# nicoRomeroCuruchet/DynamicProgramming

Hardware: AMD Instinct MI355X
Metric: state-action Bellman backups/sec (higher is better)
Workload: dtype f32; 1 GPU; double_pendulum_swingup 4D grid bins=80/dim (40960000 states) x 11 actions, gamma=0.999; step = 10 eval sweeps + 1 improve sweep = 860160000 backups; terminal states are counted in `value` (0 of 40960000: value_nonterminal leaves them out); states=40960000, nonterminal_states=40960000, actions=11, parallelism=state-range shards x1

## Files before the change

### dynamicprogramming_amd/_native.py

```python
from __future__ import annotations

import ctypes
import enum
import os
from pathlib import Path

import numpy as np

_PKG = Path(__file__).resolve().parent
LIB_PATH = _PKG / "libpi_mi355.so"
KERNEL_CACHE = Path(os.environ.get("PI_MI355_KERNEL_CACHE", str(_PKG / "_kcache")))

_f32p = ctypes.POINTER(ctypes.c_float)
_i32p = ctypes.POINTER(ctypes.c_int32)
_vp = ctypes.c_void_p

SIGNATURES = {
    "pi_abi_version": (ctypes.c_int, []),
    "pi_last_error": (ctypes.c_char_p, []),
    "pi_create": (_vp, [ctypes.c_int, ctypes.c_int, _i32p, _f32p, _f32p,
                        ctypes.POINTER(_f32p), _f32p, ctypes.c_int]),
    "pi_destroy": (None, [_vp]),
    "pi_compile": (ctypes.c_int, [_vp, ctypes.c_char_p, ctypes.c_char_p, ctypes.c_char_p,
                                  ctypes.c_size_t]),
# ... 63 lines not shown
ABI_VERSION = 12
_lib = None
_load_error: Exception | None = None


class Info(enum.IntEnum):
    N_STATES = 0
    N_ACTIONS = 1
    DIMS = 2
    EVAL_CPW = 3
    EVAL_VGPRS = 4
    IMPROVE_VGPRS = 5
    COMPUTE_UNITS = 6
    CACHE_HIT = 7
    IMPROVE_CPW = 8
    CACHED_GRAPHS = 9
    GRAPHS_ENABLED = 10
    EVAL_BLOCK = 11
    IMPROVE_BLOCK = 12
    RESIDENT_STATES_PER_THREAD = 13
    RESIDENT_ENABLED = 14
    DEBUG_CHECKS = 15
    LIVE_STATES = 16
    EVAL_LIST_ENTRIES = 17
    MEMORY_ORDER = 18
    FLOW_WORKGROUPS = 19
    RECIPROCAL_DIV = 20
    XCD_ENABLED = 30
    XCD_EVALUATIONS = 31
    XCD_FALLBACKS = 32
    WHOLE_RUNS = 33
    WHOLE_RUN_AVAILABLE = 34
    STRIP_STATES = 35


class Option(enum.IntEnum):
    EVAL_CPW = 0
    IMPROVE_CPW = 1
    GRAPHS = 2
    RESIDENT = 3
    MEMORY_ORDER = 4
    BUILD_PUSH = 5
    KEEP_LIVE_LIST = 6
    STRIP_STATES = 7
    XCD_RUN_FAILED = 8


class XcdFailure(enum.IntEnum):
    COUNT = 1
    SWITCH_OFF = 2


class CommInfo(enum.IntEnum):
    RANK = 0
    WORLD = 1
    TRANSPORT = 2
    PLAN = 3
    REACH_UNITS = 4
    ROW_EXACT = 5
    FUSED = 6
    PAIR_EXACT = 7
    FUSED_VALUES = 8
    FIRST_ENTRIES = 9
    INTERIOR_ENTRIES = 10


class Transport(enum.IntEnum):
    RCCL = 1
    IN_PROCESS = 2
    P2P = 3


class Plan(enum.IntEnum):
    NONE = 0
    ALLGATHER = 1
    HALO = 2


# ... 417 lines not shown
```

### dynamicprogramming_amd/csrc/pi_api.cpp

```cpp

#include "pi_internal.h"

#include <algorithm>
#include <cstdlib>

namespace pi {

static thread_local std::string g_error;

int fail(const std::string& msg) {
    g_error = msg;
    return 1;
}
const std::string& last_error() { return g_error; }

int env_int(const char* name, int dflt, int lo, int hi) {
    if (const char* e = std::getenv(name)) {
        const int v = std::atoi(e);
        if (v >= lo && v <= hi) return v;
    }
    return dflt;
}

void resolve_strip(pi_handle* h) {
    if (h->strip_mode >= 0) { h->strip_states = h->strip_mode; return; }
    h->strip_states = 0;
    if (h->D == 6 && h->n_states >= (int64_t(1) << 24)) {
        const int64_t sub = h->n_states / ((int64_t)h->shape[0] * h->shape[1]);
        h->strip_states = sub * std::max<int64_t>(1, ((int64_t(1) << 21) + sub / 2) / sub);
    }
}

void drop_graphs(pi_handle* h) {
    for (auto& g : h->graphs)
        if (g.exec) (void)hipGraphExecDestroy(g.exec);
    h->graphs.clear();
}

unsigned launch_blocks(int block, int64_t count, int cpw) {
    const int64_t chunks = (count + block - 1) / block;
    const int64_t groups = (chunks + cpw - 1) / cpw;
    const int64_t span = (groups + kXcds - 1) / kXcds;
    return (unsigned)std::max<int64_t>(span * kXcds, kXcds);
}

Grid2 plan_launch(const pi_handle* h, int block, int64_t first, int64_t count, int64_t total, int cpw, Sched* sc) {
    sc->cpw = cpw;
    sc->period = sc->phase = 0u;
    const int64_t group = (int64_t)block * cpw;
    const int64_t groups = ((count + block - 1) / block + cpw - 1) / cpw;
    if (h->strip_states > 0 && total > 0) {
        const double units = (double)h->strip_states * ((double)total / (double)h->n_states);
        const int64_t T = (int64_t)(units / (double)group + 0.5);
        if (T >= 16 && T < (int64_t(1) << 24) && groups > T) {
            const int64_t seg = (T + kXcds - 1) / kXcds;
            const int64_t phase = (first / group) % T;
            const int64_t periods = (groups + phase + T - 1) / T;
            if (periods <= 65535 && periods * T < (int64_t(1) << 31)) {
                sc->period = (unsigned)T;
                sc->phase = (unsigned)phase;
                return Grid2{(unsigned)(seg * kXcds), (unsigned)periods};
            }
        }
    }
    return Grid2{launch_blocks(block, count, cpw), 1u};
}

}

using namespace pi;

namespace {

unsigned int* delta_slots(pi_handle* h) { return h->d_slots; }
unsigned int* changed_slots(pi_handle* h) { return h->d_slots + kSlots; }

int zero_outputs(float* d_delta, uint32_t* d_changed, hipStream_t st) {
    if (d_delta) PI_HIP(hipMemsetAsync(d_delta, 0, sizeof(float), st));
    if (d_changed) PI_HIP(hipMemsetAsync(d_changed, 0, sizeof(uint32_t), st));
    return 0;
}

void free_device_state(pi_handle* h) {
    drop_graphs(h);
    if (h->module) (void)hipModuleUnload(h->module);
    if (h->module_push) (void)hipModuleUnload(h->module_push);
    for (void* p : {(void*)h->d_tab, (void*)h->d_slots, (void*)h->d_live, (void*)h->d_eval_list, (void*)h->d_eval_cursor,
                    h->d_flow, h->d_xcd})
        if (p) (void)hipFree(p);
}

int allocate_device_state(pi_handle* h) {
    h->num_cu = 256;
    if (h->device < 0) return 0;
    pi::DeviceGuard guard(h->device);
    hipDeviceProp_t prop;
    hipError_t e = hipGetDeviceProperties(&prop, h->device);
    if (e == hipSuccess && std::string(prop.gcnArchName).rfind(pi::kArch, 0) != 0)
        return fail(std::string("pi_create: device is ") + prop.gcnArchName + ", this library is built for gfx950 only");
    if (e == hipSuccess) e = hipMalloc((void**)&h->d_tab, h->tab.size() * sizeof(float));
    if (e == hipSuccess) e = hipMemcpy(h->d_tab, h->tab.data(), h->tab.size() * sizeof(float), hipMemcpyHostToDevice);
    if (e == hipSuccess) e = hipMalloc((void**)&h->d_slots, 2 * kSlots * sizeof(unsigned int));
    if (e == hipSuccess) e = hipMemset(h->d_slots, 0, 2 * kSlots * sizeof(unsigned int));
    if (e != hipSuccess) {
        free_device_state(h);
        return fail(std::string("pi_create: ") + hipGetErrorString(e));
    }
    h->num_cu = prop.multiProcessorCount;
    return 0;
}

void choose_dispatch(pi_handle* h) {
    const int D = h->D;
    const int64_t n = h->n_states;
    const bool big = D <= 4 && n >= (int64_t(1) << 24);
    auto block_knob = [](const char* name, int dflt) {
        const int v = env_int(name, dflt, 256, 1024);
        return (v % 64 == 0) ? v : dflt;
    };
    h->block_eval = block_knob("PI_MI355_EVAL_BLOCK", big ? 1024 : 256);
    h->block_improve = block_knob("PI_MI355_IMPROVE_BLOCK", big ? 512 : 256);
// ... 11 lines not shown
    h->resident_block = D == 2 ? 1024 : 512;
    h->resident_k = (n <= resident_max && env_int("PI_MI355_RESIDENT", 1, 0, 1))
                        ? (int)((n + h->resident_block - 1) / h->resident_block) : 0;
    const bool one_launch = env_int("PI_MI355_RESIDENT", 1, 0, 1) != 0 && env_int("PI_MI355_FLOW", 1, 0, 1) != 0;
    const bool xcd_wanted = one_launch && D == 2 && n <= (int64_t)env_int("PI_MI355_XCD_MAX", 1 << 16, 1 << 12, 1 << 17) && env_int("PI_MI355_XCD", 1, 0, 1) != 0;
    const int64_t flow_min = xcd_wanted ? std::min<int64_t>(resident_max, env_int("PI_MI355_XCD_MIN", 4096, 1024, 12288)) : resident_max;
    const int64_t flow_max = D <= 4 ? (int64_t(1) << 17) : 0;
    h->flow = one_launch && n > flow_min && n <= flow_max;
    h->xcd = h->flow && xcd_wanted;
    h->xcd_ring = env_int("PI_MI355_XCD_RING", 64, 4, 1024);
    h->xcd_states = (int)(((n + 31) / 32 + 31) / 32 * 32);
}

int build_eval_graph(pi_handle* h, float* Va, float* Vb, const int32_t* policy, const uint8_t* term,
                     int64_t s_begin, int64_t s_end, float gamma, int n_sweeps, float* d_delta,
                     hipGraphExec_t* out) {
    hipGraph_t graph;
    PI_HIP(hipGraphCreate(&graph, 0));
    hipGraphNode_t prev = nullptr;
    int rc = 0;
    for (int i = 0; i < n_sweeps && !rc; ++i)
        rc = pi::launch_eval(h, (i & 1) ? Vb : Va, (i & 1) ? Va : Vb, policy, term, s_begin, s_end, gamma,
                             i == n_sweeps - 1 && d_delta, pi::LaunchTo(graph, &prev), i >= 1);
    if (!rc) rc = pi::finalize(h, d_delta, nullptr, pi::LaunchTo(graph, &prev));
    if (!rc && hipGraphInstantiate(out, graph, nullptr, nullptr, 0) != hipSuccess) rc = 1;
    (void)hipGraphDestroy(graph);
    if (rc) {
        (void)hipGetLastError();
        return fail("could not build the evaluation-sweep graph");
    }
    return 0;
}

}

int pi::check_ready(const pi_handle* h) {
    if (!h) return fail("null handle");
    if (h->device < 0) return fail("host-only handle (device = -1) cannot launch kernels");
    if (!h->module) return fail("pi_compile has not been called on this handle");
    return 0;
}

int pi::check_range(const pi_handle* h, int64_t s_begin, int64_t s_end) {
    if (s_begin < 0 || s_end < s_begin || s_end > h->n_states)
        return fail("state range [" + std::to_string(s_begin) + ", " + std::to_string(s_end) +
                    ") outside [0, " + std::to_string(h->n_states) + ")");
    return 0;
}

int pi::finalize(pi_handle* h, float* d_delta, uint32_t* d_changed, LaunchTo to) {
    if (!d_delta && !d_changed) return 0;
    PI_HIP(launch(h->f_finalize, {1, 1}, 64, to, d_delta ? delta_slots(h) : (unsigned int*)nullptr, d_delta,
                  d_changed ? changed_slots(h) : (unsigned int*)nullptr, d_changed));
    return 0;
}

int pi::launch_eval(pi_handle* h, const float* V, float* Vnew, const int32_t* policy, const uint8_t* term,
                int64_t s_begin, int64_t s_end, float gamma, bool want_delta, LaunchTo to, bool keep_terminals) {
    if (s_end == s_begin) return 0;
    Sched sc;
    const Grid2 blocks = plan_launch(h, h->block_eval, s_begin, s_end - s_begin, h->n_states, h->cpw_eval, &sc);
    PI_HIP(launch(h->f_eval, blocks, h->block_eval, to, V, Vnew, policy, term, (const float*)h->d_tab, (long long)s_begin,
                  (long long)s_end, gamma, want_delta ? delta_slots(h) : (unsigned int*)nullptr, sc, keep_terminals ? 1 : 0));
    return 0;
}

// ... 70 lines not shown
    if (!h) return;
    if (h->device >= 0) {
        pi::DeviceGuard guard(h->device);
        pi::release_comm(h);
        free_device_state(h);
    }
    delete h;
}

int pi_eval_sweep(pi_handle* h, const float* V, float* Vnew, const int32_t* policy,
                  const uint8_t* term, int64_t s_begin, int64_t s_end, float gamma,
                  float* d_delta, void* stream) {
    if (check_ready(h) || check_range(h, s_begin, s_end)) return 1;
    if (!V || !Vnew || !policy) return fail("null device pointer");
    if (V == Vnew) return fail("V and Vnew must be different buffers (Jacobi sweep)");
    pi::DeviceGuard guard(h->device);
    hipStream_t st = (hipStream_t)stream;
    if (s_end == s_begin) return zero_outputs(d_delta, nullptr, st);
    if (pi::launch_eval(h, V, Vnew, policy, term, s_begin, s_end, gamma, d_delta != nullptr, st)) return 1;
    return pi::finalize(h, d_delta, nullptr, st);
}

int pi_eval_sweeps(pi_handle* h, float* Va, float* Vb, const int32_t* policy,
                   const uint8_t* term, int64_t s_begin, int64_t s_end, float gamma,
                   int n_sweeps, float* d_delta, void* stream) {
    if (check_ready(h) || check_range(h, s_begin, s_end)) return 1;
    if (n_sweeps < 0) return fail("n_sweeps < 0");
    if (!Va || !Vb || !policy) return fail("null device pointer");
    if (Va == Vb) return fail("Va and Vb must be different buffers (Jacobi sweep)");
    if (n_sweeps == 0) return 0;
    pi::DeviceGuard guard(h->device);
    hipStream_t st = (hipStream_t)stream;
    if (s_end == s_begin) return zero_outputs(d_delta, nullptr, st);
    if (h->f_resident && h->use_resident && n_sweeps >= 2 && s_begin == 0 && s_end == h->n_states) {
        PI_HIP(launch(h->f_resident, {1, 1}, h->resident_block, st, Va, Vb, policy, term, (const float*)h->d_tab, gamma, n_sweeps,
                      d_delta,  0.0,  1,  (int*)nullptr,  (float*)nullptr));
        return 0;
    }
    if (h->use_graphs && n_sweeps >= 4 && s_end - s_begin <= (int64_t(1) << 20)) {
        pi::GraphEntry* hit = nullptr;
        for (auto& g : h->graphs)
            if (g.Va == Va && g.Vb == Vb && g.policy == policy && g.term == term &&
                g.d_delta == d_delta && g.s_begin == s_begin && g.s_end == s_end &&
                g.gamma == gamma && g.n_sweeps == n_sweeps)
                hit = &g;
        if (!hit) {
            hipGraphExec_t exec = nullptr;
            if (build_eval_graph(h, Va, Vb, policy, term, s_begin, s_end, gamma, n_sweeps, d_delta, &exec)) {
                h->use_graphs = false;
            } else {
                if (h->graphs.size() >= 16) {
                    auto lru = std::min_element(h->graphs.begin(), h->graphs.end(),
                                                [](const GraphEntry& a, const GraphEntry& b) { return a.stamp < b.stamp; });
                    (void)hipGraphExecDestroy(lru->exec);
                    h->graphs.erase(lru);
                }
                h->graphs.push_back({Va, Vb, policy, term, d_delta, s_begin, s_end, gamma, n_sweeps, exec, 0});
                hit = &h->graphs.back();
            }
        }
        if (hit) {
            hit->stamp = ++h->graph_clock;
            PI_HIP(hipGraphLaunch(hit->exec, st));
            return 0;
        }
    }
// ... 113 lines not shown
            if (v != 0) return fail("memory order: too many digits");
            std::vector<int32_t> shape(h->D);
            std::vector<float> lo(h->D), span(h->D), rcp(h->D), tab(h->tab.begin(), h->tab.begin() + h->n_actions);
            std::vector<int> fastdiv(h->D);
            std::vector<size_t> off(h->D);
            size_t at = (size_t)h->n_actions;
            for (int d = 0; d < h->D; ++d) { off[d] = at; at += (size_t)h->shape[d]; }
            for (int k = 0; k < h->D; ++k) {
                const int d = perm[k];
                shape[k] = h->shape[d]; lo[k] = h->lo[d]; span[k] = h->span[d]; rcp[k] = h->rcp[d]; fastdiv[k] = h->fastdiv[d];
                tab.insert(tab.end(), h->tab.begin() + off[d], h->tab.begin() + off[d] + h->shape[d]);
                h->mem_of_user[d] = k;
            }
            h->user_of_mem = perm;
            h->shape = shape; h->lo = lo; h->span = span; h->rcp = rcp; h->fastdiv = fastdiv; h->tab = tab;
            if (h->device >= 0) {
                pi::DeviceGuard guard(h->device);
                PI_HIP(hipMemcpy(h->d_tab, h->tab.data(), h->tab.size() * sizeof(float), hipMemcpyHostToDevice));
            }
            return 0;
        }
        case PI_OPTION_BUILD_PUSH:
            if (value == 0) return 0;
            return pi::ensure_push_module(h);
        case PI_OPTION_KEEP_LIVE_LIST:
            h->live_force = value != 0;
            return 0;
        case PI_OPTION_STRIP_STATES:
            if (value < -1 || value > h->n_states) return fail("strip period must be -1 (auto), 0 (off) or a number of states <= n");
            h->strip_mode = value;
            resolve_strip(h);
            drop_graphs(h);
            return 0;
        case PI_OPTION_XCD_RUN_FAILED:
            if (value != PI_XCD_FAILURE_COUNT && value != PI_XCD_FAILURE_SWITCH_OFF)
                return fail("option 8 takes 1 (count a failed whole run) or 2 (and switch the XCD-local kernel off)");
            if (++h->xcd_failed >= 2 || value == PI_XCD_FAILURE_SWITCH_OFF) h->xcd_off = true;
            return 0;
        default:
            return fail("unknown option");
    }
}

int pi_debug_report(pi_handle* h, uint32_t* out4) {
    if (pi::check_ready(h)) return 1;
    if (!out4) return fail("null argument");
    if (!h->debug_bounds) return fail("this handle's kernels were built without the checks: set PI_MI355_DEBUG=1 before pi_create");
    pi::DeviceGuard guard(h->device);
    hipDeviceptr_t words = nullptr;
    size_t bytes = 0;
    PI_HIP(hipModuleGetGlobal(&words, &bytes, h->module, "pi_debug_words"));
    if (bytes != 4 * sizeof(uint32_t)) return fail("pi_debug_words has an unexpected size");
    PI_HIP(hipDeviceSynchronize());
    PI_HIP(hipMemcpy(out4, words, bytes, hipMemcpyDeviceToHost));
    PI_HIP(hipMemset(words, 0, bytes));
    return 0;
}

int64_t pi_info(pi_handle* h, int what) {
    if (!h) return -1;
    switch (what) {
        case PI_INFO_N_STATES: return h->n_states;
        case PI_INFO_N_ACTIONS: return h->n_actions;
        case PI_INFO_DIMS: return h->D;
        case PI_INFO_EVAL_CPW: return h->cpw_eval;
        case PI_INFO_EVAL_VGPRS: return h->vgpr_eval;
        case PI_INFO_IMPROVE_VGPRS: return h->vgpr_improve;
        case PI_INFO_COMPUTE_UNITS: return h->num_cu;
        case PI_INFO_CACHE_HIT: return h->cache_hit ? 1 : 0;
        case PI_INFO_IMPROVE_CPW: return h->cpw_improve;
        case PI_INFO_CACHED_GRAPHS: return (int64_t)h->graphs.size();
        case PI_INFO_GRAPHS_ENABLED: return h->use_graphs ? 1 : 0;
        case PI_INFO_EVAL_BLOCK: return h->block_eval;
        case PI_INFO_IMPROVE_BLOCK: return h->block_improve;
        case PI_INFO_RESIDENT_STATES_PER_THREAD: return h->resident_k;
        case PI_INFO_RESIDENT_ENABLED: return h->use_resident ? 1 : 0;
        case PI_INFO_DEBUG_CHECKS: return h->debug_bounds ? 1 : 0;
        case PI_INFO_LIVE_STATES: return h->live_count;
        case PI_INFO_EVAL_LIST_ENTRIES: return h->eval_count < 0 ? 0 : h->eval_count;
        case PI_INFO_MEMORY_ORDER: {
            int64_t code = 0;
            for (int k = h->D - 1; k >= 0; --k) code = (code << 3) | h->user_of_mem[k];
            return code;
        }
        case PI_INFO_FLOW_WORKGROUPS:
            return h->f_flow ? (h->n_states + h->flow_block - 1) / h->flow_block : (h->flow && h->device < 0 ? 1 : 0);
        case PI_INFO_XCD_ENABLED: return h->f_xcd && !h->xcd_off ? 1 : 0;
        case PI_INFO_XCD_EVALUATIONS: return h->xcd_used;
        case PI_INFO_XCD_FALLBACKS: return h->xcd_failed;
        case PI_INFO_WHOLE_RUNS: return h->whole_runs;
        case PI_INFO_WHOLE_RUN_AVAILABLE: return (h->f_run_resident && h->use_resident) || (h->f_xcd && !h->xcd_off) ? 1 : 0;
        case PI_INFO_STRIP_STATES: return h->strip_states;
        default:
            if (what >= PI_INFO_RECIPROCAL_DIV && what < PI_INFO_RECIPROCAL_DIV + h->D)
                return h->fastdiv[what - PI_INFO_RECIPROCAL_DIV];
            return -1;
    }
}

}
```

### dynamicprogramming_amd/csrc/pi_compile.cpp

```cpp

#include "pi_internal.h"

#include <hip/hiprtc.h>

#include <cmath>
#include <cstdio>
#include <cstdlib>
#include <algorithm>
#include <cstring>
#include <fstream>
#include <map>
#include <mutex>
#include <sstream>
#include <sys/stat.h>
#include <unistd.h>

#ifndef PI_CSRC_DIR
#error "build with -DPI_CSRC_DIR=\"...\" and -DPI_INCLUDE_DIR=\"...\""
#endif
asm(".section .rodata\n"
    ".global pi_embedded_kernels\n"
    "pi_embedded_kernels:\n"
    ".incbin \"" PI_CSRC_DIR "/pi_sweep_kernels.hip\"\n"
    ".byte 0\n"
    ".global pi_embedded_onelaunch\n"
    "pi_embedded_onelaunch:\n"
    ".incbin \"" PI_CSRC_DIR "/pi_onelaunch_kernels.hip\"\n"
    ".byte 0\n"
    ".global pi_embedded_math\n"
    "pi_embedded_math:\n"
    ".incbin \"" PI_INCLUDE_DIR "/pi_math.h\"\n"
    ".byte 0\n"
    ".global pi_embedded_push\n"
    "pi_embedded_push:\n"
    ".incbin \"" PI_CSRC_DIR "/pi_push_kernels.hip\"\n"
    ".byte 0\n"
    ".text\n");

using pi::env_int;
using pi::fail;
using pi::kXcds;

namespace {

const char* const kCompileFlags[] = {"--offload-arch=gfx950", "-O3", "-ffp-contract=off",
                                     "-std=c++17"};

uint64_t fnv1a(const std::string& s, uint64_t h) {
    for (unsigned char c : s) {
        h ^= c;
        h *= 1099511628211ull;
    }
    return h;
}

float bits_to_float(uint32_t u) {
    float f;
    std::memcpy(&f, &u, 4);
    return f;
}
// ... 50 lines not shown
std::string build_source(const pi_handle* h, const char* dynamics_src) {
    std::ostringstream o;
    auto dec = [](int x) { return std::to_string(x); };
    auto list = [](const auto& v, auto fmt) { return pi::brace_list(v.data(), v.size(), fmt); };
    o << "// generated by libpi_mi355 for " << pi::kArch << "\n";
    o << "#define PI_BLOCK_EVAL " << h->block_eval << "\n";
    o << "#define PI_BLOCK_IMPROVE " << h->block_improve << "\n";
    o << "#define PI_RESIDENT_K " << h->resident_k << "\n";
    o << "#define PI_RESIDENT_BLOCK " << h->resident_block << "\n";
    if (h->flow) o << "#define PI_FLOW 1\n#define PI_FLOW_BLOCK " << h->flow_block << "\n";
    if (h->xcd) o << "#define PI_XCD 1\n#define PI_XCD_S " << h->xcd_states << "\n#define PI_XCD_RING " << h->xcd_ring
                  << "\n#define PI_XCD_HOST_CTL_WORDS " << pi::kXcdCtlWords << "\n";
    if (h->xcd && std::getenv("PI_MI355_XCD_FIRST_SLEEP")) o << "#define PI_XCD_FIRST_SLEEP " << env_int("PI_MI355_XCD_FIRST_SLEEP", 8, 0, 127) << "\n";
    if (h->xcd && std::getenv("PI_MI355_XCD_TIMING")) o << "#define PI_XCD_TIMING 1\n";
    if (h->debug_bounds) o << "#define PI_DEBUG_BOUNDS 1\n";
    o << "#define PI_D " << h->D << "\n";
    o << "#define PI_NA " << h->n_actions << "\n";
    o << "#define PI_GRID_INIT " << list(h->shape, dec) << "\n";
    o << "#define PI_LO_INIT " << list(h->lo, pi::hex_float) << "\n";
    o << "#define PI_SPAN_INIT " << list(h->span, pi::hex_float) << "\n";
    o << "#define PI_RCP_INIT " << list(h->rcp, pi::hex_float) << "\n";
    o << "#define PI_FASTDIV_INIT " << list(h->fastdiv, dec) << "\n";
    o << "#define PI_MEM_OF_INIT " << list(h->mem_of_user, dec) << "\n";
    o << pi_embedded_math << "\n";
    o << "#define sinf pi_sinf\n#define cosf pi_cosf\n#define fmodf pi_fmodf\n";
    o << "// ---- env plugin (user string) ----\n";
    o << dynamics_src << "\n";
    o << "// ---- sweep kernels ----\n";
    o << pi_embedded_kernels << "\n";
    if (h->resident_k > 0 || h->flow || h->xcd) {
        o << "// ---- one-launch kernels ----\n";
        o << pi_embedded_onelaunch << "\n";
    }
    return o.str();
}

int load_module(pi_handle* h, const std::vector<char>& image) {
    if (h->device < 0) return 0;
    pi::DeviceGuard guard(h->device);
    pi::drop_graphs(h);
    if (h->module) {
        PI_HIP(hipModuleUnload(h->module));
        h->module = nullptr;
    }
    if (h->module_push) {
        PI_HIP(hipModuleUnload(h->module_push));
        h->module_push = nullptr;
        h->f_eval_push = nullptr;
        h->f_reach_pairs = nullptr;
    }
    PI_HIP(hipModuleLoadData(&h->module, image.data()));
    PI_HIP(hipModuleGetFunction(&h->f_eval, h->module, "pi_eval_sweep_kernel"));
    PI_HIP(hipModuleGetFunction(&h->f_eval_live, h->module, "pi_eval_live_kernel"));
    PI_HIP(hipModuleGetFunction(&h->f_policy_list, h->module, "pi_policy_list_kernel"));
    PI_HIP(hipModuleGetFunction(&h->f_scan_slots, h->module, "pi_scan_slots_kernel"));
    PI_HIP(hipModuleGetFunction(&h->f_mask_list, h->module, "pi_mask_list_kernel"));
    PI_HIP(hipModuleGetFunction(&h->f_improve, h->module, "pi_improve_sweep_kernel"));
    PI_HIP(hipModuleGetFunction(&h->f_improve_live, h->module, "pi_improve_live_kernel"));
    PI_HIP(hipModuleGetFunction(&h->f_value, h->module, "pi_value_sweep_kernel"));
    PI_HIP(hipModuleGetFunction(&h->f_finalize, h->module, "pi_finalize_kernel"));
    PI_HIP(hipModuleGetFunction(&h->f_reach_planes, h->module, "pi_reach_planes_kernel"));
    PI_HIP(hipModuleGetFunction(&h->f_reach_units, h->module, "pi_reach_units_kernel"));
    PI_HIP(hipModuleGetFunction(&h->f_probe_step, h->module, "pi_probe_step_kernel"));
    PI_HIP(hipModuleGetFunction(&h->f_probe_interp, h->module, "pi_probe_interp_kernel"));
    PI_HIP(hipModuleGetFunction(&h->f_probe_coords, h->module, "pi_probe_coords_kernel"));
    h->f_run_resident = nullptr;
    if (h->resident_k > 0) {
        PI_HIP(hipModuleGetFunction(&h->f_resident, h->module, "pi_eval_resident_kernel"));
        PI_HIP(hipModuleGetFunction(&h->f_run_resident, h->module, "pi_run_resident_kernel"));
    }
    h->f_flow = h->f_flow_finish = nullptr;
    if (h->flow) {
        PI_HIP(hipModuleGetFunction(&h->f_flow, h->module, "pi_eval_flow_kernel"));
        PI_HIP(hipModuleGetFunction(&h->f_flow_finish, h->module, "pi_flow_finish_kernel"));
        int per_cu = 0;
        const int64_t wgs = (h->n_states + h->flow_block - 1) / h->flow_block;
        if (hipModuleOccupancyMaxActiveBlocksPerMultiprocessor(&per_cu, h->f_flow, h->flow_block, 0) != hipSuccess ||
            (int64_t)(per_cu * 3 / 4) * h->num_cu < wgs) {
            (void)hipGetLastError();
            h->f_flow = nullptr;
        }
    }
    h->f_xcd = h->f_xcd_finish = nullptr;
    if (h->xcd && h->f_flow) {
        PI_HIP(hipModuleGetFunction(&h->f_xcd, h->module, "pi_xcd_kernel"));
        PI_HIP(hipModuleGetFunction(&h->f_xcd_finish, h->module, "pi_xcd_finish_kernel"));
        int regs = 0, lds = 0;
        const int64_t wgs = (h->n_states + h->xcd_states - 1) / h->xcd_states, cus = h->num_cu / kXcds, per_cu = 1;
        const bool ok = hipFuncGetAttribute(&regs, HIP_FUNC_ATTRIBUTE_NUM_REGS, h->f_xcd) == hipSuccess &&
                        hipFuncGetAttribute(&lds, HIP_FUNC_ATTRIBUTE_SHARED_SIZE_BYTES, h->f_xcd) == hipSuccess &&
                        wgs <= cus && lds > 80 * 1024 && lds <= 160 * 1024 && regs <= 128;
        if (std::getenv("PI_MI355_XCD_TRACE"))
            std::fprintf(stderr, "[pi] xcd kernel: regs %d lds %d wgs %lld cus %lld per_cu %lld ok %d\n", regs, lds, (long long)wgs,
                         (long long)cus, (long long)per_cu, (int)ok);
        if (!ok) {
            (void)hipGetLastError();
            h->f_xcd = nullptr;
        }
    }
    int v = 0;
    if (hipFuncGetAttribute(&v, HIP_FUNC_ATTRIBUTE_NUM_REGS, h->f_eval) == hipSuccess) h->vgpr_eval = v;
    if (hipFuncGetAttribute(&v, HIP_FUNC_ATTRIBUTE_NUM_REGS, h->f_improve) == hipSuccess)
        h->vgpr_improve = v;
    return 0;
}

}

namespace pi {

int ensure_push_module(pi_handle* h) {
    if (h->f_eval_push) return 0;
    if (!h->compiled || h->dynamics_src.empty()) return fail("ensure_push_module: pi_compile has not run on this handle");
    std::vector<char> image;
    const std::string src = build_source(h, h->dynamics_src.c_str()) + "// ---- fused swept-first kernel ----\n" + pi_embedded_push + "\n";
    if (compile_image(src, h->has_cache_dir ? h->cache_dir.c_str() : nullptr, nullptr, 0, image, nullptr)) return 1;
    if (h->device < 0) return 0;
    DeviceGuard guard(h->device);
    PI_HIP(hipModuleLoadData(&h->module_push, image.data()));
    PI_HIP(hipModuleGetFunction(&h->f_eval_push, h->module_push, "pi_eval_push_kernel"));
    if (h->D >= 3) PI_HIP(hipModuleGetFunction(&h->f_reach_pairs, h->module_push, "pi_reach_pairs_kernel"));
    return 0;
}

int compile_image(const std::string& src, const char* cache_dir, char* log, size_t log_len,
                  std::vector<char>& image, bool* cache_hit) {
    std::string flags;
    for (const char* f : kCompileFlags) { flags += f; flags += ' '; }
    int rtc_major = 0, rtc_minor = 0;
    (void)hiprtcVersion(&rtc_major, &rtc_minor);
    flags += "hiprtc-" + std::to_string(rtc_major) + "." + std::to_string(rtc_minor);
    char name[64];
    std::snprintf(name, sizeof name, "pi_%016llx%016llx.hsaco",
                  (unsigned long long)fnv1a(src + flags, 14695981039346656037ull),
                  (unsigned long long)fnv1a(flags + src, 0x9e3779b97f4a7c15ull));
    std::string path;
    if (cache_hit) *cache_hit = false;
    if (cache_dir && cache_dir[0]) {
        path = std::string(cache_dir) + "/" + name;
        std::ifstream f(path, std::ios::binary);
        if (f) {
            image.assign((std::istreambuf_iterator<char>(f)), std::istreambuf_iterator<char>());
            if (!image.empty()) {
                if (cache_hit) *cache_hit = true;
                return 0;
            }
        }
    }
    hiprtcProgram prog;
    if (hiprtcCreateProgram(&prog, src.c_str(), "pi_sweep_kernels.hip", 0, nullptr, nullptr) !=
        HIPRTC_SUCCESS)
        return fail("hiprtcCreateProgram failed");
    const int n_flags = (int)(sizeof kCompileFlags / sizeof kCompileFlags[0]);
    hiprtcResult rc = hiprtcCompileProgram(prog, n_flags, const_cast<const char**>(kCompileFlags));
    size_t ls = 0;
// ... 64 lines not shown
```

### dynamicprogramming_amd/csrc/pi_internal.h

```cpp
#pragma once

#include "pi_mi355.h"

#include <hip/hip_runtime.h>

#include <cstdint>
#include <memory>
#include <string>
#include <vector>

namespace pi {

int fail(const std::string& msg);
const std::string& last_error();

#define PI_HIP(expr)                                                                      \
    do {                                                                                  \
        hipError_t e_ = (expr);                                                           \
        if (e_ != hipSuccess)                                                             \
            return ::pi::fail(std::string(#expr) + ": " + hipGetErrorString(e_));         \
    } while (0)

constexpr int kProbeBlock = 256;
constexpr int kXcds = 8;
// ... 50 lines not shown
    int rank = 0, world = 1;
    virtual ~Comm() {}
    virtual int transport() const = 0;
    virtual int group_begin() = 0;
    virtual int send(const void* p, size_t bytes, int peer, hipStream_t st) = 0;
    virtual int recv(void* p, size_t bytes, int peer, hipStream_t st) = 0;
    virtual int group_end(hipStream_t st) = 0;
    virtual int allgather(void* full, size_t bytes, hipStream_t st) = 0;
    virtual int allreduce_max_f32(float* d, hipStream_t st) = 0;
    virtual int allreduce_sum_u32(uint32_t* d, hipStream_t st) = 0;
    virtual void give_up() {}
    virtual bool can_push() const { return false; }
    virtual int push_begin(const std::vector<int>&, const std::vector<int>&, float*, float* const**, hipStream_t) { return 1; }
    virtual int push_signal(hipStream_t) { return 1; }
    virtual int push_wait(hipStream_t) { return 1; }
    virtual int push_wait_deferred(hipStream_t st) { return push_wait(st); }
};
struct ShardPlan;
struct P2pPending;

struct GraphEntry {
    const void *Va = nullptr, *Vb = nullptr, *policy = nullptr, *term = nullptr, *d_delta = nullptr;
    int64_t s_begin = 0, s_end = 0;
    float gamma = 0.0f;
    int n_sweeps = 0;
    hipGraphExec_t exec = nullptr;
    uint64_t stamp = 0;
};

}

extern "C" const char pi_embedded_kernels[];
extern "C" const char pi_embedded_onelaunch[];
extern "C" const char pi_embedded_math[];
extern "C" const char pi_embedded_push[];
extern "C" const char pi_embedded_rollout[];

struct pi_handle {
    int device = -1;
    int D = 0;
    int n_actions = 0;
    int64_t n_states = 0;
    std::vector<int32_t> shape;
    std::vector<float> lo, span, rcp;
    std::vector<int> fastdiv;
    std::vector<int> mem_of_user, user_of_mem;
    bool compiled = false;
    std::vector<float> tab;
    float* d_tab = nullptr;
    unsigned int* d_slots = nullptr;
    hipModule_t module = nullptr;
    hipModule_t module_push = nullptr;
    hipFunction_t f_eval_push = nullptr, f_reach_pairs = nullptr;
    std::string dynamics_src, cache_dir;
    bool has_cache_dir = false;
    hipFunction_t f_eval = nullptr, f_eval_live = nullptr, f_policy_list = nullptr, f_scan_slots = nullptr, f_mask_list = nullptr, f_improve = nullptr, f_improve_live = nullptr, f_value = nullptr, f_finalize = nullptr,
                  f_reach_planes = nullptr, f_reach_units = nullptr, f_probe_step = nullptr, f_probe_interp = nullptr,
                  f_probe_coords = nullptr, f_resident = nullptr, f_run_resident = nullptr;
    int num_cu = 0;
    int block_eval = 256, block_improve = 256;
    int cpw_eval = 1, cpw_improve = 1;
    int64_t strip_states = 0;
    int64_t strip_mode = -1;
    int vgpr_eval = -1, vgpr_improve = -1;
    bool cache_hit = false;
    bool debug_bounds = false;
    bool use_graphs = true;
    int resident_k = 0, resident_block = 1024;
    bool use_resident = true;
    bool flow = false;
    int flow_block = 256;
    hipFunction_t f_flow = nullptr, f_flow_finish = nullptr;
    void* d_flow = nullptr;
    size_t flow_bytes = 0;
    bool xcd = false, xcd_off = false;
    int xcd_states = 1024;
    int xcd_ring = 64;
    hipFunction_t f_xcd = nullptr, f_xcd_finish = nullptr;
    void* d_xcd = nullptr;
    size_t xcd_bytes = 0;
    int64_t xcd_used = 0, xcd_failed = 0, whole_runs = 0;
    unsigned int* xcd_ctl = nullptr;
    std::vector<pi::GraphEntry> graphs;
    uint64_t graph_clock = 0;
    const uint8_t* live_term = nullptr;
    int32_t* d_live = nullptr;
    int64_t live_count = 0;
    bool live_force = false;
    int64_t live_lo = 0, live_hi = 0;
    int32_t* d_eval_list = nullptr;
    unsigned long long* d_eval_cursor = nullptr;
    int64_t eval_count = -1;
    const int32_t* eval_policy = nullptr;
    std::vector<const float*> eval_holds;
    std::vector<uint64_t> live_bits;
    std::vector<int64_t> live_before;
    pi::Comm* comm = nullptr;
    pi::ShardPlan* plan = nullptr;
    pi::P2pPending* p2p_pending = nullptr;
};

struct pi_infer {
    int device = -1;
    int D = 0;
    int64_t n_corners = 0, n_states = 0;
    int n_actions = 0;
    hipModule_t module = nullptr;
    hipFunction_t f = nullptr;
    float* d_actions = nullptr;
    int32_t* d_policy = nullptr;
    std::string grid_defines, cache_dir;
    bool has_cache_dir = false;
    hipModule_t module_rollout = nullptr;
    hipFunction_t f_rollout = nullptr;
    bool has_dynamics = false;
    std::string dynamics_src;
    std::vector<int32_t> corner_bits;
    hipModule_t module_hybrid = nullptr;
    hipFunction_t f_hybrid = nullptr;
    bool has_partner = false;
    std::string partner_defines;
};

namespace pi {

int check_ready(const pi_handle* h);
int check_range(const pi_handle* h, int64_t s_begin, int64_t s_end);
int launch_eval(pi_handle* h, const float* V, float* Vnew, const int32_t* policy, const uint8_t* term,
                int64_t s_begin, int64_t s_end, float gamma, bool want_delta, LaunchTo to,
                bool keep_terminals = false);
int finalize(pi_handle* h, float* d_delta, uint32_t* d_changed, LaunchTo to);
bool live_usable(const pi_handle* h, const uint8_t* term, int64_t s_begin, int64_t s_end);
void live_span(const pi_handle* h, int64_t s_begin, int64_t s_end, int64_t* first, int64_t* count);
void live_states(const pi_handle* h, int64_t s_begin, int64_t s_end, std::vector<int32_t>& out);
int launch_eval_live(pi_handle* h, const float* V, float* Vnew, const int32_t* policy, int64_t first, int64_t count,
                     float gamma, bool want_delta, hipStream_t st, const int32_t* list = nullptr, int64_t list_total = 0);
int64_t live_list_total(const pi_handle* h, int64_t entries);
struct Sched {
    int cpw;
    unsigned int period, phase;
};
Grid2 plan_launch(const pi_handle* h, int block, int64_t first, int64_t count, int64_t total, int cpw, Sched* sc);
int ensure_push_module(pi_handle* h);
unsigned launch_blocks(int block, int64_t count, int cpw);
int launch_eval_push(pi_handle* h, const float* V, float* Vnew, const int32_t* policy, const int32_t* list,
                     const uint8_t* dest, float* const* d_peers, int n_peers, int64_t count, float gamma, bool want_delta,
                     hipStream_t st);
bool pairs_possible(const pi_handle* h);
int reach_pairs(pi_handle* h, const uint8_t* term, int64_t s_begin, int64_t s_end, uint32_t* d_bitmap, hipStream_t st);
void drop_eval_list(pi_handle* h);
void release_comm(pi_handle* h);
void drop_p2p_pending(pi_handle* h);
double comm_timeout_seconds();
void drop_graphs(pi_handle* h);
void resolve_strip(pi_handle* h);
bool validate_fast_division(float span);
int compile_image(const std::string& src, const char* cache_dir, char* log, size_t log_len,
                  std::vector<char>& image, bool* cache_hit);
int check_rollout_args(int D, const float* d_start, int64_t m, int n_steps, const float* d_final, const float* d_traj,
                       int traj_every, int64_t* blocks);
int drop_hybrid(pi_infer* h);

}
```

### dynamicprogramming_amd/csrc/pi_live.cpp

```cpp

#include "pi_internal.h"

#include <algorithm>

using pi::env_int;
using pi::fail;

namespace pi {

bool live_usable(const pi_handle* h, const uint8_t* term, int64_t s_begin, int64_t s_end) {
    return h->live_count > 0 && term != nullptr && term == h->live_term && s_begin >= h->live_lo && s_end <= h->live_hi;
}

void live_span(const pi_handle* h, int64_t s_begin, int64_t s_end, int64_t* first, int64_t* count) {
    const int64_t word0 = h->live_lo >> 6;
    auto position = [&](int64_t s) {
        if (s <= h->live_lo) return int64_t(0);
        if (s >= h->live_hi) return h->live_count;
        const uint64_t word = h->live_bits[(size_t)((s >> 6) - word0)];
        const uint64_t below = (s & 63) ? word & ((uint64_t(1) << (s & 63)) - 1) : 0;
        return h->live_before[(size_t)((s >> 6) - word0)] + (int64_t)__builtin_popcountll(below);
    };
    *first = position(s_begin);
    *count = position(s_end) - *first;
}

void live_states(const pi_handle* h, int64_t s_begin, int64_t s_end, std::vector<int32_t>& out) {
    const int64_t a = std::max(s_begin, h->live_lo), b = std::min(s_end, h->live_hi);
    const int64_t word0 = h->live_lo >> 6;
    for (int64_t w = a >> 6; w <= (b - 1) >> 6 && a < b; ++w) {
        uint64_t word = h->live_bits[(size_t)(w - word0)];
        while (word) {
            const int bit = __builtin_ctzll(word);
            word &= word - 1;
            const int64_t s = (w << 6) + bit;
            if (s >= a && s < b) out.push_back((int32_t)s);
        }
    }
}

int64_t live_list_total(const pi_handle* h, int64_t entries) {
    const int64_t range = h->live_hi - h->live_lo;
    if (range <= 0 || entries <= 0) return 0;
    return (int64_t)((double)entries * ((double)h->n_states / (double)range));
}

void drop_eval_list(pi_handle* h) {
    h->eval_count = -1;
    h->eval_policy = nullptr;
    h->eval_holds.clear();
}

}

namespace {

template <typename Pass>
hipError_t count_and_scan(pi_handle* h, Pass pass, long long nblocks, unsigned long long* slots, hipStream_t st,
                          unsigned long long* total) {
    hipError_t err = pass(0);
    if (err == hipSuccess) err = pi::launch(h->f_scan_slots, {1, 1}, 1024, st, slots, nblocks);
    if (err == hipSuccess) err = hipMemcpyAsync(total, slots + nblocks, sizeof *total, hipMemcpyDeviceToHost, st);
    if (err == hipSuccess) err = hipStreamSynchronize(st);
    return err;
}

}

extern "C" {

int pi_prepare_mask(pi_handle* h, const uint8_t* d_term, void* stream) {
    if (pi::check_ready(h)) return 1;
    return pi_prepare_mask_range(h, d_term, 0, h->n_states, stream);
}

int pi_prepare_mask_range(pi_handle* h, const uint8_t* d_term, int64_t s_begin, int64_t s_end, void* stream) {
    if (pi::check_ready(h) || pi::check_range(h, s_begin, s_end)) return 1;
    pi::DeviceGuard guard(h->device);
    if (h->d_live) { (void)hipFree(h->d_live); h->d_live = nullptr; }
    if (h->d_eval_list) { (void)hipFree(h->d_eval_list); h->d_eval_list = nullptr; }
    if (h->d_eval_cursor) { (void)hipFree(h->d_eval_cursor); h->d_eval_cursor = nullptr; }
    pi::drop_eval_list(h);
    h->live_term = nullptr;
// ... 42 lines not shown
        return fail(std::string("pi_prepare_mask: ") + hipGetErrorString(err));
    }
    std::vector<int64_t> before_block(nwords + 1, 0);
    for (size_t k = 0; k < nwords; ++k) before_block[k + 1] = before_block[k] + (int64_t)__builtin_popcountll(bits[k]);
    if (before_block[nwords] != n_live) {
        (void)hipFree(h->d_live);
        h->d_live = nullptr;
        return fail("pi_prepare_mask: the bitmap and the list disagree");
    }
    h->live_term = d_term;
    h->live_lo = s_begin;
    h->live_hi = s_end;
    h->live_count = n_live;
    h->live_bits = std::move(bits);
    h->live_before = std::move(before_block);
    return 0;
}

int64_t pi_live_list(pi_handle* h, int32_t* d_out, int64_t capacity, void* stream) {
    if (pi::check_ready(h)) return -1;
    if (h->live_count <= 0 || !h->d_live) return 0;
    if (!d_out) return h->live_count;
    if (capacity < h->live_count) { fail("pi_live_list: capacity below the list's length"); return -1; }
    pi::DeviceGuard guard(h->device);
    if (hipMemcpyAsync(d_out, h->d_live, (size_t)h->live_count * sizeof(int32_t), hipMemcpyDeviceToDevice,
                       (hipStream_t)stream) != hipSuccess) { fail("pi_live_list: copy failed"); return -1; }
    return h->live_count;
}

int pi_eval_begin(pi_handle* h, const int32_t* policy, const uint8_t* term, void* stream) {
    if (pi::check_ready(h)) return 1;
    if (!policy) return fail("null device pointer");
    pi::drop_eval_list(h);
    if (!pi::live_usable(h, term, 0, h->n_states) || !env_int("PI_MI355_EVAL_LIST", 1, 0, 1)) return 0;
    pi::DeviceGuard guard(h->device);
    hipStream_t st = (hipStream_t)stream;
    const long long nblocks = (h->live_count + pi::kProbeBlock - 1) / pi::kProbeBlock;
    if (!h->d_eval_list) PI_HIP(hipMalloc((void**)&h->d_eval_list, (size_t)h->live_count * sizeof(int32_t)));
    if (!h->d_eval_cursor) PI_HIP(hipMalloc((void**)&h->d_eval_cursor, (size_t)(nblocks + 1) * sizeof(unsigned long long)));
    auto pass = [&](int which) {
        return pi::launch(h->f_policy_list, {(unsigned)nblocks, 1}, pi::kProbeBlock, st, (const int32_t*)h->d_live,
                          (long long)h->live_count, policy, (const float*)h->d_tab, h->d_eval_cursor, h->d_eval_list, which);
    };
    unsigned long long kept = 0;
    PI_HIP(count_and_scan(h, pass, nblocks, h->d_eval_cursor, st, &kept));
    PI_HIP(pass(1));
    PI_HIP(hipStreamSynchronize(st));
    if ((double)kept > 0.97 * (double)h->live_count) return 0;
    h->eval_count = (int64_t)kept;
    h->eval_policy = policy;
    return 0;
}

int pi_eval_end(pi_handle* h) {
    if (!h) return fail("null handle");
    pi::drop_eval_list(h);
    return 0;
}


}
```

### include/pi_mi355.h

```cpp
#ifndef PI_MI355_H_
#define PI_MI355_H_

#include <stddef.h>
#include <stdint.h>

#ifdef __cplusplus
extern "C" {
#endif

typedef struct pi_handle pi_handle;

#define PI_MI355_ABI_VERSION 12
int pi_abi_version(void);

const char* pi_last_error(void);

pi_handle* pi_create(int device, int D, const int32_t* grid_shape, const float* lo,
                     const float* hi, const float* const* bins, const float* actions,
                     int n_actions);
void pi_destroy(pi_handle* h);

int pi_compile(pi_handle* h, const char* dynamics_src, const char* cache_dir, char* log,
               size_t log_len);

// ... 102 lines not shown
int pi_probe_coords(pi_handle* h, int64_t s_begin, int64_t s_end, float* out, int chunks_per_workgroup,
                    void* stream);
int pi_plan_schedule(pi_handle* h, int block, int64_t first, int64_t count, int64_t total, int chunks_per_workgroup,
                     uint64_t* out6);

typedef struct pi_infer pi_infer;
pi_infer* pi_infer_create(int device, int D, const float* lo, const float* hi, const int32_t* grid_shape,
                          const int32_t* strides, const int32_t* corner_bits, int64_t n_corners,
                          const char* cache_dir);
void pi_infer_destroy(pi_infer* h);
int pi_infer_set_policy(pi_infer* h, const int32_t* policy, int64_t n_states, const float* action_space,
                        int n_actions);
int pi_infer_query(pi_infer* h, const float* d_points, int64_t m, float* d_actions_out, float* d_weights_out,
                   int32_t* d_indices_out, void* stream);
int pi_infer_set_dynamics(pi_infer* h, const char* dynamics_src, char* log, size_t log_len);
int pi_infer_rollout(pi_infer* h, const float* d_start, int64_t m, int n_steps, float gamma, float* d_final,
                     float* d_return, int32_t* d_length, uint8_t* d_terminated, float* d_traj, int traj_every,
                     void* stream);
int pi_infer_set_partner(pi_infer* h, pi_infer* partner, char* log, size_t log_len);
int pi_infer_rollout_hybrid(pi_infer* h, pi_infer* partner, const float* d_start, int64_t m, int n_steps, float gamma,
                            const float* enter, const float* leave, float* d_final, float* d_return, int32_t* d_length,
                            uint8_t* d_terminated, int32_t* d_secondary_steps, uint8_t* d_last_mode, float* d_traj,
                            int traj_every, void* stream);

enum pi_option_code {
    PI_OPTION_EVAL_CPW = 0,
    PI_OPTION_IMPROVE_CPW = 1,
    PI_OPTION_GRAPHS = 2,
    PI_OPTION_RESIDENT = 3,
    PI_OPTION_MEMORY_ORDER = 4,
    PI_OPTION_BUILD_PUSH = 5,
    PI_OPTION_KEEP_LIVE_LIST = 6,
    PI_OPTION_STRIP_STATES = 7,
    PI_OPTION_XCD_RUN_FAILED = 8
};
enum pi_xcd_failure {
    PI_XCD_FAILURE_COUNT = 1,
    PI_XCD_FAILURE_SWITCH_OFF = 2
};
int pi_set_option(pi_handle* h, int what, int64_t value);

enum pi_info_code {
    PI_INFO_N_STATES = 0,
    PI_INFO_N_ACTIONS = 1,
    PI_INFO_DIMS = 2,
    PI_INFO_EVAL_CPW = 3,
    PI_INFO_EVAL_VGPRS = 4,
    PI_INFO_IMPROVE_VGPRS = 5,
    PI_INFO_COMPUTE_UNITS = 6,
    PI_INFO_CACHE_HIT = 7,
    PI_INFO_IMPROVE_CPW = 8,
    PI_INFO_CACHED_GRAPHS = 9,
    PI_INFO_GRAPHS_ENABLED = 10,
    PI_INFO_EVAL_BLOCK = 11,
    PI_INFO_IMPROVE_BLOCK = 12,
    PI_INFO_RESIDENT_STATES_PER_THREAD = 13,
    PI_INFO_RESIDENT_ENABLED = 14,
    PI_INFO_DEBUG_CHECKS = 15,
    PI_INFO_LIVE_STATES = 16,
    PI_INFO_EVAL_LIST_ENTRIES = 17,
    PI_INFO_MEMORY_ORDER = 18,
    PI_INFO_FLOW_WORKGROUPS = 19,
    PI_INFO_RECIPROCAL_DIV = 20,
    PI_INFO_XCD_ENABLED = 30,
    PI_INFO_XCD_EVALUATIONS = 31,
    PI_INFO_XCD_FALLBACKS = 32,
    PI_INFO_WHOLE_RUNS = 33,
    PI_INFO_WHOLE_RUN_AVAILABLE = 34,
    PI_INFO_STRIP_STATES = 35
};
int64_t pi_info(pi_handle* h, int what);

int pi_debug_report(pi_handle* h, uint32_t* out4);

#ifdef __cplusplus
}
#endif
#endif
```

Measured before the change: 144.2 billion backups/s.

## Sort each block's states by successor cell for ordered evaluation sweeps

Adds a build kernel that, for the current policy, computes each state's successor grid cell and bitonic-sorts the states within each block by that cell. It stores a 16-bit permutation entry (lane plus action) and a count of non-terminal states per block. Later evaluation sweeps visit states in this order, so neighbouring lanes gather nearby V entries and terminal states are packed at the end. The goal is better cache locality for the interpolation gathers and less wave divergence. The cost is the build kernel, an extra permutation read per state each sweep, and scattered writes to Vn. The path turns on automatically for 4D grids with at least 2^24 states, and the permutation is reused for as long as the same policy is being evaluated.

Result: no change. 144.1 billion backups/s (-0.0%).

```diff
diff --git a/dynamicprogramming_amd/_native.py b/dynamicprogramming_amd/_native.py
--- a/dynamicprogramming_amd/_native.py
+++ b/dynamicprogramming_amd/_native.py
@@ -119,6 +119,7 @@
     WHOLE_RUNS = 33
     WHOLE_RUN_AVAILABLE = 34
     STRIP_STATES = 35
+    EVAL_ORDERED = 37
 
 
 class Option(enum.IntEnum):
@@ -131,6 +132,7 @@
     KEEP_LIVE_LIST = 6
     STRIP_STATES = 7
     XCD_RUN_FAILED = 8
+    EVAL_ORDER = 9
 
 
 class XcdFailure(enum.IntEnum):
diff --git a/dynamicprogramming_amd/csrc/pi_api.cpp b/dynamicprogramming_amd/csrc/pi_api.cpp
--- a/dynamicprogramming_amd/csrc/pi_api.cpp
+++ b/dynamicprogramming_amd/csrc/pi_api.cpp
@@ -29,6 +29,15 @@
         const int64_t sub = h->n_states / ((int64_t)h->shape[0] * h->shape[1]);
         h->strip_states = sub * std::max<int64_t>(1, ((int64_t(1) << 21) + sub / 2) / sub);
     }
+}
+
+bool order_possible(const pi_handle* h) {
+    return h->n_actions <= 64 && h->block_eval <= 1024 && (h->block_eval & (h->block_eval - 1)) == 0 &&
+           h->tab.size() * sizeof(float) <= 48 * 1024;
+}
+bool order_wanted(const pi_handle* h) {
+    if (!order_possible(h) || h->order_mode == 0) return false;
+    return h->order_mode == 1 || (h->D == 4 && h->n_states >= (int64_t(1) << 24));
 }
 
 void drop_graphs(pi_handle* h) {
@@ -86,7 +95,7 @@
     if (h->module) (void)hipModuleUnload(h->module);
     if (h->module_push) (void)hipModuleUnload(h->module_push);
     for (void* p : {(void*)h->d_tab, (void*)h->d_slots, (void*)h->d_live, (void*)h->d_eval_list, (void*)h->d_eval_cursor,
-                    h->d_flow, h->d_xcd})
+                    (void*)h->d_order, h->d_flow, h->d_xcd})
         if (p) (void)hipFree(p);
 }
 
@@ -164,6 +173,26 @@
     return 0;
 }
 
+constexpr int kOrderMinSweeps = 29;
+
+int build_order(pi_handle* h, const int32_t* policy, const uint8_t* term, hipStream_t st) {
+    const int64_t chunks = (h->n_states + h->block_eval - 1) / h->block_eval;
+    if (!h->d_order) PI_HIP(hipMalloc((void**)&h->d_order, (size_t)(chunks * h->block_eval + chunks) * sizeof(uint16_t)));
+    PI_HIP(launch(h->f_order_build, {(unsigned)chunks, 1}, h->block_eval, st, policy, term, (const float*)h->d_tab,
+                  (long long)h->n_states, h->d_order, h->d_order + chunks * h->block_eval));
+    return 0;
+}
+
+int launch_eval_ordered(pi_handle* h, const float* V, float* Vnew, float gamma, bool want_delta, hipStream_t st) {
+    const int64_t chunks = (h->n_states + h->block_eval - 1) / h->block_eval;
+    Sched sc;
+    const Grid2 blocks = plan_launch(h, h->block_eval, 0, h->n_states, h->n_states, h->cpw_eval, &sc);
+    PI_HIP(launch(h->f_eval_ordered, blocks, h->block_eval, st, V, Vnew, (const uint16_t*)h->d_order,
+                  (const uint16_t*)(h->d_order + chunks * h->block_eval), (const float*)h->d_tab, (long long)h->n_states, gamma,
+                  want_delta ? delta_slots(h) : (unsigned int*)nullptr, sc));
+    return 0;
+}
+
 }
 
 int pi::check_ready(const pi_handle* h) {
@@ -300,6 +329,25 @@
     pi::DeviceGuard guard(h->device);
     hipStream_t st = (hipStream_t)stream;
     if (s_end == s_begin) return zero_outputs(d_delta, nullptr, st);
+    h->last_batch_ordered = 0;
+    if (h->f_eval_ordered && n_sweeps >= 2 && s_begin == 0 && s_end == h->n_states && !pi::live_usable(h, term, s_begin, s_end)) {
+        const bool bracket = h->order_bracket && policy == h->order_policy && term == h->order_term;
+        if (bracket || h->order_mode == 1 || n_sweeps >= kOrderMinSweeps) {
+            const bool reuse = bracket && h->order_valid;
+            if (!reuse && build_order(h, policy, term, st)) return 1;
+            if (bracket) h->order_valid = true;
+            for (int i = 0; i < n_sweeps; ++i) {
+                const float* src = (i & 1) ? Vb : Va;
+                float* dst = (i & 1) ? Va : Vb;
+                const bool want = i == n_sweeps - 1 && d_delta != nullptr;
+                if (i == 0 ? pi::launch_eval(h, src, dst, policy, term, s_begin, s_end, gamma, want, st, false)
+                           : launch_eval_ordered(h, src, dst, gamma, want, st))
+                    return 1;
+            }
+            h->last_batch_ordered = reuse ? 2 : 1;
+            return pi::finalize(h, d_delta, nullptr, st);
+        }
+    }
     if (h->f_resident && h->use_resident && n_sweeps >= 2 && s_begin == 0 && s_end == h->n_states) {
         PI_HIP(launch(h->f_resident, {1, 1}, h->resident_block, st, Va, Vb, policy, term, (const float*)h->d_tab, gamma, n_sweeps,
                       d_delta,  0.0,  1,  (int*)nullptr,  (float*)nullptr));
@@ -479,6 +527,16 @@
             resolve_strip(h);
             drop_graphs(h);
             return 0;
+        case PI_OPTION_EVAL_ORDER: {
+            if (value < -1 || value > 1) return fail("the evaluation order is -1 (auto), 0 (off) or 1 (on)");
+            const bool before = pi::order_wanted(h);
+            h->order_mode = value;
+            h->order_valid = false;
+            if (pi::order_wanted(h) == before) return 0;
+            pi::DeviceGuard guard(h->device);
+            if (h->device >= 0 && h->compiled) PI_HIP(hipDeviceSynchronize());
+            return pi::reload_module(h);
+        }
         case PI_OPTION_XCD_RUN_FAILED:
             if (value != PI_XCD_FAILURE_COUNT && value != PI_XCD_FAILURE_SWITCH_OFF)
                 return fail("option 8 takes 1 (count a failed whole run) or 2 (and switch the XCD-local kernel off)");
@@ -538,6 +596,7 @@
         case PI_INFO_WHOLE_RUNS: return h->whole_runs;
         case PI_INFO_WHOLE_RUN_AVAILABLE: return (h->f_run_resident && h->use_resident) || (h->f_xcd && !h->xcd_off) ? 1 : 0;
         case PI_INFO_STRIP_STATES: return h->strip_states;
+        case PI_INFO_EVAL_ORDERED: return h->last_batch_ordered;
         default:
             if (what >= PI_INFO_RECIPROCAL_DIV && what < PI_INFO_RECIPROCAL_DIV + h->D)
                 return h->fastdiv[what - PI_INFO_RECIPROCAL_DIV];
diff --git a/dynamicprogramming_amd/csrc/pi_compile.cpp b/dynamicprogramming_amd/csrc/pi_compile.cpp
--- a/dynamicprogramming_amd/csrc/pi_compile.cpp
+++ b/dynamicprogramming_amd/csrc/pi_compile.cpp
@@ -26,6 +26,10 @@
     ".global pi_embedded_onelaunch\n"
     "pi_embedded_onelaunch:\n"
     ".incbin \"" PI_CSRC_DIR "/pi_onelaunch_kernels.hip\"\n"
+    ".byte 0\n"
+    ".global pi_embedded_order\n"
+    "pi_embedded_order:\n"
+    ".incbin \"" PI_CSRC_DIR "/pi_order_kernels.hip\"\n"
     ".byte 0\n"
     ".global pi_embedded_math\n"
     "pi_embedded_math:\n"
@@ -142,6 +146,10 @@
         o << "// ---- one-launch kernels ----\n";
         o << pi_embedded_onelaunch << "\n";
     }
+    if (pi::order_wanted(h)) {
+        o << "// ---- ordered evaluation kernels ----\n";
+        o << pi_embedded_order << "\n";
+    }
     return o.str();
 }
 
@@ -179,6 +187,11 @@
         PI_HIP(hipModuleGetFunction(&h->f_resident, h->module, "pi_eval_resident_kernel"));
         PI_HIP(hipModuleGetFunction(&h->f_run_resident, h->module, "pi_run_resident_kernel"));
     }
+    h->f_order_build = h->f_eval_ordered = nullptr;
+    if (pi::order_wanted(h)) {
+        PI_HIP(hipModuleGetFunction(&h->f_order_build, h->module, "pi_order_build_kernel"));
+        PI_HIP(hipModuleGetFunction(&h->f_eval_ordered, h->module, "pi_eval_ordered_kernel"));
+    }
     h->f_flow = h->f_flow_finish = nullptr;
     if (h->flow) {
         PI_HIP(hipModuleGetFunction(&h->f_flow, h->module, "pi_eval_flow_kernel"));
@@ -231,6 +244,15 @@
     PI_HIP(hipModuleGetFunction(&h->f_eval_push, h->module_push, "pi_eval_push_kernel"));
     if (h->D >= 3) PI_HIP(hipModuleGetFunction(&h->f_reach_pairs, h->module_push, "pi_reach_pairs_kernel"));
     return 0;
+}
+
+int reload_module(pi_handle* h) {
+    if (!h->compiled || h->dynamics_src.empty()) return 0;
+    std::vector<char> image;
+    if (compile_image(build_source(h, h->dynamics_src.c_str()), h->has_cache_dir ? h->cache_dir.c_str() : nullptr, nullptr, 0,
+                      image, &h->cache_hit))
+        return 1;
+    return load_module(h, image);
 }
 
 int compile_image(const std::string& src, const char* cache_dir, char* log, size_t log_len,
diff --git a/dynamicprogramming_amd/csrc/pi_internal.h b/dynamicprogramming_amd/csrc/pi_internal.h
--- a/dynamicprogramming_amd/csrc/pi_internal.h
+++ b/dynamicprogramming_amd/csrc/pi_internal.h
@@ -106,6 +106,7 @@
 
 extern "C" const char pi_embedded_kernels[];
 extern "C" const char pi_embedded_onelaunch[];
+extern "C" const char pi_embedded_order[];
 extern "C" const char pi_embedded_math[];
 extern "C" const char pi_embedded_push[];
 extern "C" const char pi_embedded_rollout[];
@@ -167,6 +168,13 @@
     int64_t eval_count = -1;
     const int32_t* eval_policy = nullptr;
     std::vector<const float*> eval_holds;
+    int64_t order_mode = -1;
+    hipFunction_t f_order_build = nullptr, f_eval_ordered = nullptr;
+    uint16_t* d_order = nullptr;
+    bool order_bracket = false, order_valid = false;
+    const int32_t* order_policy = nullptr;
+    const uint8_t* order_term = nullptr;
+    int last_batch_ordered = 0;
     std::vector<uint64_t> live_bits;
     std::vector<int64_t> live_before;
     pi::Comm* comm = nullptr;
@@ -223,6 +231,9 @@
 bool pairs_possible(const pi_handle* h);
 int reach_pairs(pi_handle* h, const uint8_t* term, int64_t s_begin, int64_t s_end, uint32_t* d_bitmap, hipStream_t st);
 void drop_eval_list(pi_handle* h);
+bool order_possible(const pi_handle* h);
+bool order_wanted(const pi_handle* h);
+int reload_module(pi_handle* h);
 void release_comm(pi_handle* h);
 void drop_p2p_pending(pi_handle* h);
 double comm_timeout_seconds();
diff --git a/dynamicprogramming_amd/csrc/pi_live.cpp b/dynamicprogramming_amd/csrc/pi_live.cpp
--- a/dynamicprogramming_amd/csrc/pi_live.cpp
+++ b/dynamicprogramming_amd/csrc/pi_live.cpp
@@ -49,6 +49,9 @@
     h->eval_count = -1;
     h->eval_policy = nullptr;
     h->eval_holds.clear();
+    h->order_bracket = h->order_valid = false;
+    h->order_policy = nullptr;
+    h->order_term = nullptr;
 }
 
 }
@@ -157,6 +160,9 @@
     if (pi::check_ready(h)) return 1;
     if (!policy) return fail("null device pointer");
     pi::drop_eval_list(h);
+    h->order_bracket = true;
+    h->order_policy = policy;
+    h->order_term = term;
     if (!pi::live_usable(h, term, 0, h->n_states) || !env_int("PI_MI355_EVAL_LIST", 1, 0, 1)) return 0;
     pi::DeviceGuard guard(h->device);
     hipStream_t st = (hipStream_t)stream;
diff --git a/dynamicprogramming_amd/csrc/pi_order_kernels.hip b/dynamicprogramming_amd/csrc/pi_order_kernels.hip
--- /dev/null
+++ b/dynamicprogramming_amd/csrc/pi_order_kernels.hip
@@ -0,0 +1,119 @@
+
+#define PI_ORDER_LANE_BITS 10
+#define PI_ORDER_LANE_MASK ((1u << PI_ORDER_LANE_BITS) - 1u)
+static_assert(PI_BLOCK_EVAL <= (1 << PI_ORDER_LANE_BITS), "a lane offset has 10 bits");
+static_assert((PI_BLOCK_EVAL & (PI_BLOCK_EVAL - 1)) == 0, "the bitonic network needs a power of two");
+static_assert(PI_NA <= 64, "an action has 6 bits");
+
+#define PI_ORDER_KEY_DONE ((1u << 22) - 2u)
+#define PI_ORDER_KEY_PARKED ((1u << 22) - 1u)
+constexpr int pi_order_shift() {
+    int s = 0;
+    while (((PI_GRID.n - 1) >> s) >= (long long)PI_ORDER_KEY_DONE) ++s;
+    return s;
+}
+#define PI_ORDER_SHIFT pi_order_shift()
+
+extern "C" __global__ void __launch_bounds__(PI_BLOCK_EVAL)
+pi_order_build_kernel(const int* __restrict__ policy, const unsigned char* __restrict__ term,
+                      const float* __restrict__ tab, long long n, unsigned short* __restrict__ perm,
+                      unsigned short* __restrict__ counts) {
+    __shared__ float lds_tab[PI_GRID.tab_len];
+    __shared__ unsigned int words[2][PI_BLOCK_EVAL];
+    __shared__ unsigned char acts[PI_BLOCK_EVAL];
+    pi_stage_table<PI_BLOCK_EVAL>(tab, lds_tab);
+    __syncthreads();
+    const unsigned int tid = threadIdx.x;
+    const long long cb = (long long)blockIdx.x * PI_BLOCK_EVAL;
+    const long long s = cb + tid;
+    unsigned int key = PI_ORDER_KEY_PARKED;
+    int action = 0;
+    if (s < n && !(term != nullptr && term[s])) {
+        action = pi_checked_action(policy[s], (unsigned int)s);
+        float x[PI_D], ns[PI_D], reward;
+        pi_state_coords((unsigned int)s, lds_tab, x);
+        bool done;
+        pi_dynamics(x, lds_tab[PI_TAB_ACT + action], ns, &reward, &done);
+        key = PI_ORDER_KEY_DONE;
+        if (!done) {
+            unsigned int base;
+            float fr[PI_D];
+            pi_locate(ns, base, fr);
+            key = base >> PI_ORDER_SHIFT;
+        }
+    }
+    acts[tid] = (unsigned char)(action & 63);
+    unsigned int v = (key << PI_ORDER_LANE_BITS) | tid;
+    int flip = 0;
+    for (unsigned int k = 2; k <= PI_BLOCK_EVAL; k <<= 1) {
+        for (unsigned int j = k >> 1; j > 0; j >>= 1) {
+            unsigned int o;
+            if (j >= 64u) {
+                words[flip][tid] = v;
+                __syncthreads();
+                o = words[flip][tid ^ j];
+                flip ^= 1;
+            } else {
+                o = (unsigned int)__shfl_xor((int)v, (int)j, 64);
+            }
+            const bool keep_min = ((tid & j) == 0u) == ((tid & k) == 0u);
+            v = keep_min ? min(v, o) : max(v, o);
+        }
+    }
+    __syncthreads();
+    const unsigned int lane = v & PI_ORDER_LANE_MASK;
+    const bool used = (v >> PI_ORDER_LANE_BITS) != PI_ORDER_KEY_PARKED;
+    perm[cb + tid] = (unsigned short)(lane | ((unsigned int)acts[lane] << PI_ORDER_LANE_BITS));
+    const int n_used = __syncthreads_count(used);
+    if (tid == 0) counts[blockIdx.x] = (unsigned short)n_used;
+}
+
+extern "C" __global__ void __launch_bounds__(PI_BLOCK_EVAL) __attribute__((amdgpu_num_sgpr(80)))
+pi_eval_ordered_kernel(const float* __restrict__ V, float* __restrict__ Vn, const unsigned short* __restrict__ perm,
+                       const unsigned short* __restrict__ counts, const float* __restrict__ tab, long long n,
+                       float gamma, unsigned int* __restrict__ delta_bits, PiSched sc) {
+    __shared__ float lds_tab[PI_GRID.tab_len];
+    long long chunk0, n_chunks;
+    if (!pi_first_chunk<PI_BLOCK_EVAL>(n, sc, chunk0, n_chunks)) return;
+    const int n_here = (int)(min(chunk0 + sc.cpw, n_chunks) - chunk0);
+
+    const unsigned int tid = threadIdx.x;
+    long long cb = chunk0 * PI_BLOCK_EVAL;
+    unsigned int ent_nxt = __builtin_nontemporal_load(pi_lane_ptr(perm + cb, tid));
+    unsigned int cnt_nxt = counts[chunk0];
+    pi_stage_table<PI_BLOCK_EVAL>(tab, lds_tab);
+    __syncthreads();
+
+    float dmax = 0.0f;
+    for (int k = 0; k < n_here; ++k) {
+        const unsigned int ent = ent_nxt, cnt = cnt_nxt;
+        const unsigned int s = (unsigned int)cb + (ent & PI_ORDER_LANE_MASK);
+        if (k + 1 < n_here) {
+            cb += PI_BLOCK_EVAL;
+            ent_nxt = __builtin_nontemporal_load(pi_lane_ptr(perm + cb, tid));
+            cnt_nxt = counts[chunk0 + k + 1];
+        }
+        if (tid < cnt) {
+            float v_old = 0.0f;
+            if (delta_bits != nullptr) v_old = PI_OFF32 ? *pi_lane_ptr(V, s) : V[s];
+            float x[PI_D], ns[PI_D], reward;
+            pi_state_coords(s, lds_tab, x);
+            const float a = lds_tab[PI_TAB_ACT + (int)(ent >> PI_ORDER_LANE_BITS)];
+            bool done;
+            pi_dynamics(x, a, ns, &reward, &done);
+            float e = 0.0f;
+            if (!done) {
+                unsigned int base;
+                float fr[PI_D];
+                pi_locate(ns, base, fr);
+                e = pi_interpolate(V, base, fr);
+            }
+            const float nv = reward + gamma * e;
+            if (PI_OFF32) pi_store_lane(Vn, s, nv);
+            else Vn[s] = nv;
+            const float dlt = fabsf(nv - v_old);
+            dmax = dlt > dmax ? dlt : dmax;
+        }
+    }
+    if (delta_bits != nullptr) pi_wave_max_to<PI_BLOCK_EVAL>(dmax, delta_bits);
+}
diff --git a/include/pi_mi355.h b/include/pi_mi355.h
--- a/include/pi_mi355.h
+++ b/include/pi_mi355.h
@@ -158,7 +158,8 @@
     PI_OPTION_BUILD_PUSH = 5,
     PI_OPTION_KEEP_LIVE_LIST = 6,
     PI_OPTION_STRIP_STATES = 7,
-    PI_OPTION_XCD_RUN_FAILED = 8
+    PI_OPTION_XCD_RUN_FAILED = 8,
+    PI_OPTION_EVAL_ORDER = 9
 };
 enum pi_xcd_failure {
     PI_XCD_FAILURE_COUNT = 1,
@@ -193,7 +194,8 @@
     PI_INFO_XCD_FALLBACKS = 32,
     PI_INFO_WHOLE_RUNS = 33,
     PI_INFO_WHOLE_RUN_AVAILABLE = 34,
-    PI_INFO_STRIP_STATES = 35
+    PI_INFO_STRIP_STATES = 35,
+    PI_INFO_EVAL_ORDERED = 37
 };
 int64_t pi_info(pi_handle* h, int what);
 
```
